# qc-tum/TNC

Hardware: NVIDIA H100
Metric: pairwise contractions/sec (effective ZGEMM TFLOP/s in zgemm_tflops) (higher is better)
Workload: dtype f64

## Files before the change

### tnc_b200/csrc/crt.cu

```cuda
#include "internal.h"
#include "sm90.h"
#include <cuda.h>
#include <algorithm>
#include <cmath>
#include <cstdio>
#include <cstdlib>

namespace tncb {

constexpr int CRT_MAX_MOD = 20;
static const int kModuli[CRT_MAX_MOD] = {256, 253, 251, 249, 247, 245, 241, 239, 233, 229,
                                         227, 223, 211, 199, 197, 193, 191, 181, 179, 173};
constexpr int CRT_BT = 128;
constexpr int CRT_BKB = WG_BKB;
#ifndef CRT_RING3_STAGES
#define CRT_RING3_STAGES 3
#endif
#ifndef CRT_RING3_BK
#define CRT_RING3_BK 128
#endif
#ifndef CRT_RING4_STAGES
#define CRT_RING4_STAGES 5
#endif
#ifndef CRT_RING4_BK
// ... 112 lines not shown
  unsigned long long mv[RES_ROWS_C * RES_K_C / 256];
#pragma unroll
  for (int it = 0; it < RES_ROWS_C * RES_K_C / 256; it++) {
    int r, k;
    crt_tile_coord(it * 256 + tid, lk, r, k);
    const long long orow = s_offr[r], ok = s_offk[k];
    mv[it] = 0ull;
    if (orow >= 0 && ok >= 0) {
      const double2 v = __ldg(src + orow + ok);
      mv[it] = max((unsigned long long)__double_as_longlong(fabs(v.x)), (unsigned long long)__double_as_longlong(fabs(v.y)));
    }
  }
  int cur_r = -1;
  unsigned long long cur_m = 0ull;
#pragma unroll
  for (int it = 0; it < RES_ROWS_C * RES_K_C / 256; it++) {
    int r, k;
    crt_tile_coord(it * 256 + tid, lk, r, k);
    unsigned long long m = mv[it];
    for (int d = 1; d < (1 << lk); d <<= 1) m = max(m, __shfl_xor_sync(0xffffffffu, m, d));
    if (r != cur_r) {
      if (cur_m && (tid & ((1 << lk) - 1)) == 0) atomicMax(&s_max[cur_r], cur_m);
      cur_r = r; cur_m = 0ull;
    }
    cur_m = max(cur_m, m);
  }
  if (cur_m && (tid & ((1 << lk) - 1)) == 0) atomicMax(&s_max[cur_r], cur_m);
  __syncthreads();
  if (tid < RES_ROWS_C && row0 + tid < rows && s_max[tid] != 0ull) atomicMax(rowmax + row0 + tid, s_max[tid]);
}

__device__ __forceinline__ int crt_fix_byte(int s, int m) {
  if (s > 127) s -= m;
  else if (s < -128) s += m;
  return s;
}
constexpr int RES_ROWS = RES_ROWS_C, RES_K = RES_K_C, RES_RS = RES_K + RES_K / 8 + 1;
template <int COMPS, bool KARA>
__global__ void __launch_bounds__(256, 3)
crt_residue_kernel(const double2* __restrict__ src, const long long* __restrict__ off_row, const long long* __restrict__ off_k,
                   long long rows, long long K, long long rowsP, long long Kp, const unsigned long long* __restrict__ rowmax, int bits, int lk,
                   const __grid_constant__ CrtTables T, int8_t* __restrict__ planes) {
  extern __shared__ __align__(16) unsigned char res_smem_raw[];
  double2* tile = reinterpret_cast<double2*>(res_smem_raw);
  __shared__ double s_scale[RES_ROWS];
  __shared__ long long s_offr[RES_ROWS], s_offk[RES_K];
  __shared__ double s_inv[CRT_MAX_MOD];
  __shared__ int s_mod[CRT_MAX_MOD];
  const long long row0 = (long long)blockIdx.x * RES_ROWS, k0 = (long long)blockIdx.y * RES_K;
  const int tid = threadIdx.x;
  const double two_a = scalbn(1.0, bits);
  if (tid >= 64 && tid < 64 + CRT_MAX_MOD) { s_inv[tid - 64] = T.inv_mod[tid - 64]; s_mod[tid - 64] = T.mod[tid - 64]; }
  if (tid < RES_ROWS) {
    const long long r = row0 + tid;
    const int e = r < rows ? crt_exp_from_bits(rowmax[r]) : 0;
    s_scale[tid] = (e == kExpNonFinite) ? 0.0 : scalbn(1.0, -e);
    s_offr[tid] = r < rows ? __ldg(off_row + r) : -1;
  } else if (tid >= 128) {
    const int k = tid - 128;
    s_offk[k] = k0 + k < K ? __ldg(off_k + k0 + k) : -1;
  }
  __syncthreads();
  double2 vv[RES_ROWS * RES_K / 256];
#pragma unroll
  for (int it = 0; it < RES_ROWS * RES_K / 256; it++) {
    int r, k;
    crt_tile_coord(it * 256 + tid, lk, r, k);
    const long long orow = s_offr[r], ok = s_offk[k];
    vv[it] = make_double2(0.0, 0.0);
    if (orow >= 0 && ok >= 0) vv[it] = __ldg(src + orow + ok);
  }
#pragma unroll
  for (int it = 0; it < RES_ROWS * RES_K / 256; it++) {
    int r, k;
    crt_tile_coord(it * 256 + tid, lk, r, k);
    const double sc = s_scale[r];
    double2 v = vv[it];
    v.x = trunc(v.x * sc * two_a);
    v.y = trunc(v.y * sc * two_a);
    if (sc == 0.0) { v.x = 0.0; v.y = 0.0; }
    tile[r * RES_RS + k + (k >> 3)] = v;
  }
  __syncthreads();
  const int r = tid >> 3;
  if (row0 + r >= rows) return;
  const double RMAGIC = 6755399441055744.0;
  const long long plane_stride = rowsP * Kp;
#pragma unroll 1
  for (int pass = 0; pass < 2; pass++) {
    const int g = (tid & 7) + 8 * pass;
    double xr[8], xi[8];
    int lr[8], li[8];
#pragma unroll
    for (int j = 0; j < 8; j++) {
      const double2 v = tile[r * RES_RS + g * 9 + j];
      xr[j] = v.x; xi[j] = v.y;
      lr[j] = (int)__double2ll_rn(v.x); li[j] = (int)__double2ll_rn(v.y);
    }
    int8_t* dst = planes + (row0 + r) * Kp + k0 + g * 8;
    const int nmod = T.nmod;
#pragma unroll 1
    for (int i = 0; i < nmod; i++) {
      const int m = s_mod[i];
      const double inv = s_inv[i];
      uint32_t wr[2] = {0, 0}, wi[2] = {0, 0}, ws[2] = {0, 0};
#pragma unroll
      for (int j = 0; j < 8; j++) {
        const int qr = __double2loint(fma(xr[j], inv, RMAGIC));
        const int qi = __double2loint(fma(xi[j], inv, RMAGIC));
        const int rr = lr[j] - qr * m, ri = li[j] - qi * m;
        constexpr uint32_t sel[4] = {0x3214u, 0x3240u, 0x3410u, 0x4210u};
        wr[j >> 2] = __byte_perm(wr[j >> 2], (uint32_t)rr, sel[j & 3]);
        wi[j >> 2] = __byte_perm(wi[j >> 2], (uint32_t)ri, sel[j & 3]);
        if (KARA) ws[j >> 2] = __byte_perm(ws[j >> 2], (uint32_t)crt_fix_byte(rr + ri, m), sel[j & 3]);
      }
      int8_t* d = dst + (long long)i * (KARA ? 3 : COMPS) * plane_stride;
      if (KARA) {
        *reinterpret_cast<uint2*>(d) = make_uint2(wr[0], wr[1]);
        *reinterpret_cast<uint2*>(d + plane_stride) = make_uint2(wi[0], wi[1]);
        *reinterpret_cast<uint2*>(d + 2 * plane_stride) = make_uint2(ws[0], ws[1]);
      } else if (COMPS == 2) {
        *reinterpret_cast<uint2*>(d) = make_uint2(wr[0], wr[1]);
        *reinterpret_cast<uint2*>(d + plane_stride) = make_uint2(wi[0], wi[1]);
      } else {
        *reinterpret_cast<uint2*>(d) = make_uint2(__vneg4(wi[0]), __vneg4(wi[1]));
        *reinterpret_cast<uint2*>(d + plane_stride) = make_uint2(wr[0], wr[1]);
        *reinterpret_cast<uint2*>(d + 2 * plane_stride) = make_uint2(wi[0], wi[1]);
      }
    }
  }
}

struct CrtGemmArgs {
  int8_t* R;
  int Np, Mp;
  int tiles_n, tiles_m, tile_m;
  int nmod, nkc, kb_per_chunk, num_kb;
  int total_items;
  int group;
  int negmod[CRT_MAX_MOD];
  int magic[CRT_MAX_MOD];
};

struct CrtItem { int mod_i, prod, kc, n0, m0; };
template <bool KARA>
__device__ __forceinline__ CrtItem crt_decode(const CrtGemmArgs& p, int item) {
  const int tiles = p.tiles_n * p.tiles_m;
  const int mk = item / tiles, t = item - mk * tiles;
  CrtItem it;
  const int mp = mk / p.nkc;
  it.kc = mk - mp * p.nkc;
  it.mod_i = KARA ? mp / 3 : mp; it.prod = KARA ? mp - it.mod_i * 3 : 0;
  const int per_band = p.group * p.tiles_m;
  const int band = t / per_band, first = band * p.group;
  const int gsize = min(p.group, p.tiles_n - first);
  const int r = t - band * per_band;
  it.n0 = (first + r % gsize) * CRT_BT;
  it.m0 = (r / gsize) * p.tile_m;
  return it;
}

template <bool KARA>
__global__ void __launch_bounds__(WG_THREADS, 1)
crt_gemm_kernel(const __grid_constant__ CUtensorMap mapB, const __grid_constant__ CUtensorMap mapA,
                const __grid_constant__ CrtGemmArgs p) {
  constexpr int STAGES = CrtRing<KARA>::STAGES, BK = CrtRing<KARA>::BK, SUB = CRT_BKB / BK;
  using Stage = typename CrtRing<KARA>::Stage;
  extern __shared__ __align__(1024) uint8_t crt_smem_raw[];
  uint8_t* smem = reinterpret_cast<uint8_t*>((reinterpret_cast<uintptr_t>(crt_smem_raw) + 1023) & ~(uintptr_t)1023);
  __shared__ uint64_t full_bar[STAGES], empty_bar[STAGES];
  const int wg = threadIdx.x >> 7, tid = threadIdx.x & 127;

  if (threadIdx.x == 0) {
    for (int s = 0; s < STAGES; s++) { wg_mbar_init(&full_bar[s], 1); wg_mbar_init(&empty_bar[s], 2); }
    asm volatile("fence.mbarrier_init.release.cluster;" ::: "memory");
  }
  __syncthreads();

  if (wg == 0) {
    wg_setmaxnreg_producer();
    if (tid != 0) return;
    int it = 0;
    for (int item = blockIdx.x; item < p.total_items; item += gridDim.x) {
      const CrtItem w = crt_decode<KARA>(p, item);
      const int kb0 = w.kc * p.kb_per_chunk, kb1 = min(p.num_kb, kb0 + p.kb_per_chunk);
      const int rowB = (KARA ? w.mod_i * 3 + w.prod : w.mod_i * 2) * p.Np + w.n0;
      const int rowA = (KARA ? w.mod_i * 3 + w.prod : w.mod_i * 3) * p.Mp + w.m0;
      for (int ks = kb0 * SUB; ks < kb1 * SUB; ks++, it++) {
        uint8_t* st = wg_produce_begin<STAGES, KARA, BK>(smem, full_bar, empty_bar, it);
        uint64_t* bar = &full_bar[it % STAGES];
        const int kx = ks * BK;
        uint8_t* a = st + Stage::A;
        wg_tma_2d(&mapB, bar, st, kx, rowB);
        if (KARA) {
          wg_tma_2d(&mapA, bar, a, kx, rowA);
          wg_tma_2d(&mapA, bar, a + Stage::TILE, kx, rowA + WG_ROWS);
        } else {
          wg_tma_2d(&mapB, bar, st + Stage::B1, kx, rowB + p.Np);
          wg_tma_2d(&mapA, bar, a, kx, rowA);
          wg_tma_2d(&mapA, bar, a + Stage::TILE, kx, rowA + p.Mp);
          wg_tma_2d(&mapA, bar, a + 2 * Stage::TILE, kx, rowA + 2 * p.Mp);
        }
      }
    }
  } else {
    wg_setmaxnreg_consumer();
    const int c = wg - 1, wq = tid >> 5, lane = tid & 31;
    const int q = lane & 3;
    const bool q0 = q & 1, q1 = q & 2;
    WgRing<STAGES, KARA, BK> ring{smem, full_bar, empty_bar};
    uint32_t acc[128];
#pragma unroll
    for (int i = 0; i < 128; i++) acc[i] = 0u;
    for (int item = blockIdx.x; item < p.total_items; item += gridDim.x) {
      const CrtItem w = crt_decode<KARA>(p, item);
      const int kb0 = w.kc * p.kb_per_chunk, kb1 = min(p.num_kb, kb0 + p.kb_per_chunk);
      bool first = true;
      for (int ks = kb0 * SUB; ks < kb1 * SUB; ks++) ring.mma_stage(acc, c, first, tid == 0);
      ring.drain(tid == 0);
      const int negm = p.negmod[w.mod_i], magic = p.magic[w.mod_i];
      int8_t* row_base[2];
#pragma unroll
      for (int h = 0; h < 2; h++) {
        const long long n = (long long)w.n0 + c * 64 + wq * 16 + (lane >> 2) + 8 * h;
        row_base[h] = KARA ? p.R + ((long long)((w.mod_i * p.nkc + w.kc) * 3 + w.prod) * p.Np + n) * p.Mp + w.m0
                           : p.R + ((long long)((w.mod_i * p.nkc + w.kc) * 2) * p.Np + n) * p.Mp + w.m0;
      }
#pragma unroll
      for (int i = 0; i < 4; i++) {
#pragma unroll
        for (int h = 0; h < 2; h++) {
          uint32_t x[4];
#pragma unroll
          for (int k = 0; k < 4; k++) {
            uint32_t u = 0;
#pragma unroll
            for (int jj = 0; jj < 2; jj++) {
#pragma unroll
              for (int e = 0; e < 2; e++) {
                const int a = (int)acc[4 * (8 * i + 2 * k + jj) + 2 * h + e];
                int t = __mulhi(a, magic) * negm + a;
                if (t > 127) t += negm;
                u |= (((uint32_t)t & 0xffu) ^ 0x80u) << (8 * (2 * jj + e));
              }
            }
            x[k] = u;
          }
          const uint32_t r0 = __shfl_xor_sync(0xffffffffu, q0 ? x[0] : x[1], 1);
          const uint32_t r1 = __shfl_xor_sync(0xffffffffu, q0 ? x[2] : x[3], 1);
          const uint32_t a0 = q0 ? r0 : x[0], a1 = q0 ? x[1] : r0;
          const uint32_t b0 = q0 ? r1 : x[2], b1 = q0 ? x[3] : r1;
          const uint32_t g0 = __shfl_xor_sync(0xffffffffu, q1 ? a0 : b0, 2);
          const uint32_t g1 = __shfl_xor_sync(0xffffffffu, q1 ? a1 : b1, 2);
          const uint32_t k0 = q1 ? b0 : a0, k1 = q1 ? b1 : a1;
          const uint32_t y0 = q1 ? g0 : k0, y1 = q1 ? g1 : k1, y2 = q1 ? k0 : g0, y3 = q1 ? k1 : g1;
          const uint4 v = make_uint4(__byte_perm(y0, y1, 0x5410), __byte_perm(y2, y3, 0x5410),
                                     __byte_perm(y0, y1, 0x7632), __byte_perm(y2, y3, 0x7632));
          const int cc = 4 * i + q;
          int8_t* dst = KARA ? row_base[h] + cc * 16
                             : row_base[h] + (i >= 2 ? (long long)p.Np * p.Mp : 0LL) + (cc & 7) * 16;
          *reinterpret_cast<uint4*>(dst) = v;
        }
      }
    }
  }
}

struct CrtReconArgs {
  const int8_t* R;
  double2* C;
  const unsigned long long* max_n;
  const unsigned long long* max_m;
  long long rows, cols, ldc;
  long long Np, Mp;
  int nkc;
};

template <bool ONE_CHUNK, bool KARA>
__global__ void __launch_bounds__(256, 4)
crt_reconstruct_kernel(const __grid_constant__ CrtReconArgs a, const __grid_constant__ CrtTables T) {
  const long long cols4 = a.Mp >> 2;
  const long long idx = (long long)blockIdx.x * blockDim.x + threadIdx.x;
  const long long n = idx / cols4, m4 = (idx - n * cols4) * 4;
  if (n >= a.rows || m4 >= a.cols) return;
  double s1r[4], s2r[4], s1i[4], s2i[4];
#pragma unroll
  for (int j = 0; j < 4; j++) { s1r[j] = s2r[j] = s1i[j] = s2i[j] = 0.0; }
  const long long plane = a.Np * a.Mp;
  const int8_t* base = a.R + n * a.Mp + m4;
  const double bias = 4503599627370496.0 + (KARA ? 256.0 : 128.0) * (double)a.nkc;
  const double bias_i = 4503599627370496.0 + (KARA ? 384.0 : 128.0) * (double)a.nkc;
#pragma unroll 8
  for (int i = 0; i < T.nmod; i++) {
    uint32_t ur[4], ui[4];
    if (KARA) {
#pragma unroll
      for (int j = 0; j < 4; j++) { ur[j] = 0; ui[j] = 0; }
      for (int c = 0; c < (ONE_CHUNK ? 1 : a.nkc); c++) {
        const int8_t* pk = base + (long long)((i * a.nkc + c) * 3) * plane;
        const uint32_t w1 = __ldg(reinterpret_cast<const uint32_t*>(pk));
        const uint32_t w2 = __ldg(reinterpret_cast<const uint32_t*>(pk + plane));
        const uint32_t w3 = __ldg(reinterpret_cast<const uint32_t*>(pk + 2 * plane));
#pragma unroll
        for (int j = 0; j < 4; j++) {
          const uint32_t k1 = __byte_perm(w1, 0, 0x4440 + j), k2 = __byte_perm(w2, 0, 0x4440 + j);
          ur[j] += 256u + k1 - k2;
          ui[j] += 512u + __byte_perm(w3, 0, 0x4440 + j) - k1 - k2;
        }
      }
    } else if (ONE_CHUNK) {
      const uint32_t wr = __ldg(reinterpret_cast<const uint32_t*>(base + (long long)(i * 2) * plane));
      const uint32_t wi = __ldg(reinterpret_cast<const uint32_t*>(base + (long long)(i * 2 + 1) * plane));
#pragma unroll
      for (int j = 0; j < 4; j++) { ur[j] = __byte_perm(wr, 0, 0x4440 + j); ui[j] = __byte_perm(wi, 0, 0x4440 + j); }
    } else {
#pragma unroll
      for (int j = 0; j < 4; j++) { ur[j] = 0; ui[j] = 0; }
      for (int c = 0; c < a.nkc; c++) {
        const int8_t* pr = base + (long long)((i * a.nkc + c) * 2) * plane;
        const uint32_t wr = __ldg(reinterpret_cast<const uint32_t*>(pr));
        const uint32_t wi = __ldg(reinterpret_cast<const uint32_t*>(pr + plane));
#pragma unroll
        for (int j = 0; j < 4; j++) { ur[j] += __byte_perm(wr, 0, 0x4440 + j); ui[j] += __byte_perm(wi, 0, 0x4440 + j); }
      }
    }
    const double r1 = T.rho1[i], r2 = T.rho2[i];
#pragma unroll
    for (int j = 0; j < 4; j++) {
      const double dr = __hiloint2double(0x43300000, (int)ur[j]) - bias;
      const double di = __hiloint2double(0x43300000, (int)ui[j]) - bias_i;
      s1r[j] = fma(dr, r1, s1r[j]); s2r[j] = fma(dr, r2, s2r[j]);
      s1i[j] = fma(di, r1, s1i[j]); s2i[j] = fma(di, r2, s2i[j]);
    }
  }
  const int en = crt_exp_from_bits(a.max_n[n]);
  double2* dst = a.C + n * a.ldc + m4;
  const double RMAGIC = 6755399441055744.0;
#pragma unroll
  for (int j = 0; j < 4; j++) {
    if (m4 + j >= a.cols) break;
    const int em = crt_exp_from_bits(a.max_m[m4 + j]);
    double2 out;
    if (en == kExpNonFinite || em == kExpNonFinite) {
      out = make_double2(__longlong_as_double(0x7ff8000000000000LL), __longlong_as_double(0x7ff8000000000000LL));
    } else {
      const double qr = ((s1r[j] + s2r[j]) + RMAGIC) - RMAGIC;
      const double qi = ((s1i[j] + s2i[j]) + RMAGIC) - RMAGIC;
      const double fr = (s1r[j] - qr) + s2r[j], fi = (s1i[j] - qi) + s2i[j];
      out = make_double2(scalbn(fr * T.p_scaled, en + em), scalbn(fi * T.p_scaled, en + em));
    }
    dst[j] = out;
  }
}

typedef CUresult (*EncodeTiledFn)(CUtensorMap*, CUtensorMapDataType, cuuint32_t, void*, const cuuint64_t*, const cuuint64_t*,
                                  const cuuint32_t*, const cuuint32_t*, CUtensorMapInterleave, CUtensorMapSwizzle,
                                  CUtensorMapL2promotion, CUtensorMapFloatOOBfill);
static EncodeTiledFn get_encode() {
  static EncodeTiledFn fn = nullptr;
  static bool tried = false;
  if (!tried) {
    tried = true;
    cudaDriverEntryPointQueryResult q;
    void* p = nullptr;
    if (cudaGetDriverEntryPoint("cuTensorMapEncodeTiled", &p, cudaEnableDefault, &q) == cudaSuccess) fn = (EncodeTiledFn)p;
  }
  return fn;
}
template <int BK>
int wg_make_map(CUtensorMap* m, void* ptr, uint64_t rows, uint64_t kbytes) {
  static_assert(BK == 128 || BK == 64, "SWIZZLE_128B or SWIZZLE_64B");
  EncodeTiledFn enc = get_encode();
  if (!enc) return fail(TNCB_ERR_CUDA, "cuTensorMapEncodeTiled is not available");
  cuuint64_t dims[2] = {kbytes, rows};
  cuuint64_t strides[1] = {kbytes};
  cuuint32_t box[2] = {(cuuint32_t)BK, (cuuint32_t)WG_ROWS};
  cuuint32_t estr[2] = {1, 1};
  CUresult r = enc(m, CU_TENSOR_MAP_DATA_TYPE_UINT8, 2, ptr, dims, strides, box, estr, CU_TENSOR_MAP_INTERLEAVE_NONE,
                   BK == 128 ? CU_TENSOR_MAP_SWIZZLE_128B : CU_TENSOR_MAP_SWIZZLE_64B, CU_TENSOR_MAP_L2_PROMOTION_L2_256B,
                   CU_TENSOR_MAP_FLOAT_OOB_FILL_NONE);
  if (r != CUDA_SUCCESS) return fail(TNCB_ERR_CUDA, "cuTensorMapEncodeTiled failed: " + std::to_string((int)r));
  return TNCB_OK;
}
template int wg_make_map<128>(CUtensorMap*, void*, uint64_t, uint64_t);
template int wg_make_map<64>(CUtensorMap*, void*, uint64_t, uint64_t);

static inline long long round_up_ll(long long x, long long a) { return (x + a - 1) / a * a; }


int launch_k1_crt(tncb_ctx* ctx, const PairPlan& P, const double2* A, const double2* B, double2* C,
                  const long long* offAm, const long long* offBn, const long long* offAk, const long long* offBk) {
  int nmod, bits_a, bits_b;
  const int want = ctx->crt_tol > 0.0 ? crt_bits_for_tolerance(P.K, ctx->crt_tol) : ctx->crt_bits;
  crt_choose(P.K, want, ctx->crt_nmod_force, &nmod, &bits_a, &bits_b);
  CrtTables T;
  crt_make_tables(nmod, bits_a, bits_b, T);
  cudaStream_t st = ctx->stream;
  const long long Kp = round_up_ll(P.K, CRT_BKB);
  const int num_kb = (int)(Kp / CRT_BKB);
  const int ctas_max = std::max(1, ctx->sm_count);
  const bool kara = ctx->crt_products == 3 || (ctx->crt_products == 0 && Kp >= ctx->crt_kara_min_k);
  const int TM = kara ? 2 * CRT_BT : CRT_BT;
  const int NPB = kara ? 3 : 2, NPR = kara ? 3 : 2;
  const long long tiles_total = round_up_ll(P.N, CRT_BT) / CRT_BT * (round_up_ll(P.M, TM) / TM);
  int nkc = (int)((Kp + CRT_KCHUNK_MAX - 1) / CRT_KCHUNK_MAX);
  {
    const long long items = tiles_total * nmod * (kara ? 3 : 1);
    const long long want = ctas_max;
    if (items * nkc < want) nkc = (int)std::min<long long>((want + items - 1) / items, std::max(1, num_kb / 8));
    nkc = std::max(1, std::min(nkc, 32));
  }
  int kb_per_chunk = (num_kb + nkc - 1) / nkc;
  nkc = (num_kb + kb_per_chunk - 1) / kb_per_chunk;
  if ((long long)kb_per_chunk * CRT_BKB > CRT_KCHUNK_MAX) return fail(TNCB_ERR_UNSUPPORTED, "K too long for the int8 engine");

  const size_t budget = ctx->crt_ws_bytes;
  long long pn = round_up_ll(P.N, CRT_BT), pm = round_up_ll(P.M, TM);
  auto ws_bytes = [&](long long n_, long long m_) {
    return (size_t)nmod * (size_t)Kp * (size_t)(NPB * n_ + 3 * m_) + (size_t)nmod * nkc * NPR * (size_t)n_ * (size_t)m_;
  };
  while (ws_bytes(pn, pm) > budget && (pm > TM || pn > CRT_BT)) {
    if (pm >= pn && pm > TM) pm = round_up_ll(pm / 2, TM);
    else if (pn > CRT_BT) pn = round_up_ll(pn / 2, CRT_BT);
    else pm = round_up_ll(pm / 2, TM);
  }
  const size_t bytesB = (size_t)nmod * NPB * pn * Kp, bytesA = (size_t)nmod * 3 * pm * Kp;
  const size_t bytesR = (size_t)nmod * nkc * NPR * pn * pm;
  const size_t bytesE = (size_t)(pn + pm) * sizeof(unsigned long long);
  void *pb = nullptr, *pa = nullptr, *pr = nullptr, *pe = nullptr;
  int rc;
  if ((rc = ctx->arena.alloc(bytesB, &pb))) return rc;
  if ((rc = ctx->arena.alloc(bytesA, &pa))) { ctx->arena.free(pb, bytesB); return rc; }
  if ((rc = ctx->arena.alloc(bytesR, &pr))) { ctx->arena.free(pb, bytesB); ctx->arena.free(pa, bytesA); return rc; }
  if ((rc = ctx->arena.alloc(bytesE, &pe))) { ctx->arena.free(pb, bytesB); ctx->arena.free(pa, bytesA); ctx->arena.free(pr, bytesR); return rc; }
  auto cleanup = [&]() { ctx->arena.free(pb, bytesB); ctx->arena.free(pa, bytesA); ctx->arena.free(pr, bytesR); ctx->arena.free(pe, bytesE); };
  unsigned long long* max_n = (unsigned long long*)pe;
  unsigned long long* max_m = max_n + pn;

  static bool attr_done_dev[64] = {false};
  bool& attr_done = attr_done_dev[ctx->device & 63];
  const int smem_gemm4 = CrtRing<false>::SMEM, smem_gemm3 = CrtRing<true>::SMEM;
  const int smem_res = RES_ROWS * RES_RS * (int)sizeof(double2);
  if (!attr_done) {
    cudaError_t e = cudaFuncSetAttribute(crt_gemm_kernel<false>, cudaFuncAttributeMaxDynamicSharedMemorySize, smem_gemm4);
    if (e == cudaSuccess) e = cudaFuncSetAttribute(crt_gemm_kernel<true>, cudaFuncAttributeMaxDynamicSharedMemorySize, smem_gemm3);
    if (e == cudaSuccess) e = cudaFuncSetAttribute(crt_residue_kernel<2, false>, cudaFuncAttributeMaxDynamicSharedMemorySize, smem_res);
    if (e == cudaSuccess) e = cudaFuncSetAttribute(crt_residue_kernel<3, false>, cudaFuncAttributeMaxDynamicSharedMemorySize, smem_res);
    if (e == cudaSuccess) e = cudaFuncSetAttribute(crt_residue_kernel<2, true>, cudaFuncAttributeMaxDynamicSharedMemorySize, smem_res);
    if (e == cudaSuccess) e = cudaFuncSetAttribute(crt_residue_kernel<3, true>, cudaFuncAttributeMaxDynamicSharedMemorySize, smem_res);
    if (e != cudaSuccess) { cleanup(); return fail(TNCB_ERR_CUDA, cudaGetErrorString(e)); }
    attr_done = true;
  }
  auto lane_split = [](const LegList& kl, bool k_is_b, const LegList& fl) {
    auto p2 = [](long long d) { int b = 0; while ((2LL << b) <= d && b < 5) b++; return b; };
    const long long ks = kl.n ? (k_is_b ? kl.sb[kl.n - 1] : kl.sa[kl.n - 1]) : (1LL << 62);
    const long long fs = fl.n ? fl.sa[fl.n - 1] : (1LL << 62);
    if (ks <= fs) return kl.n ? p2(kl.dim[kl.n - 1]) : 0;
    return 0;
  };
  const int lk_b = lane_split(P.k, true, P.n), lk_a = lane_split(P.k, false, P.m);
  ctx->last_int8_ops = 0.0; ctx->last_nmod = nmod; ctx->last_products = kara ? 3 : 4;
  bool timed = false;

  for (long long n0 = 0; n0 < P.N; n0 += pn) {
    const long long nrows = std::min(pn, P.N - n0);
    const long long Np = round_up_ll(nrows, CRT_BT);
    if (Np != nrows) cudaMemsetAsync(pb, 0, (size_t)nmod * NPB * Np * Kp, st);
    cudaMemsetAsync(max_n, 0, (size_t)nrows * sizeof(unsigned long long), st);
    {
      dim3 g((unsigned)((nrows + RES_ROWS - 1) / RES_ROWS), (unsigned)(Kp / RES_K));
      crt_rowmax_kernel<<<g, 256, 0, st>>>(B, offBn + n0, offBk, nrows, P.K, lk_b, max_n);
      if (kara) crt_residue_kernel<2, true><<<g, 256, smem_res, st>>>(B, offBn + n0, offBk, nrows, P.K, Np, Kp, max_n, bits_b, lk_b, T, (int8_t*)pb);
      else crt_residue_kernel<2, false><<<g, 256, smem_res, st>>>(B, offBn + n0, offBk, nrows, P.K, Np, Kp, max_n, bits_b, lk_b, T, (int8_t*)pb);
    }
    ctx->launches += 2;
    CUtensorMap mapB;
    if ((rc = kara ? wg_make_map<CrtRing<true>::BK>(&mapB, pb, (uint64_t)nmod * NPB * Np, (uint64_t)Kp)
                   : wg_make_map<CrtRing<false>::BK>(&mapB, pb, (uint64_t)nmod * NPB * Np, (uint64_t)Kp))) { cleanup(); return rc; }
    for (long long m0 = 0; m0 < P.M; m0 += pm) {
      const long long mcols = std::min(pm, P.M - m0);
      const long long Mp = round_up_ll(mcols, TM);
      if (Mp != mcols) cudaMemsetAsync(pa, 0, (size_t)nmod * 3 * Mp * Kp, st);
      cudaMemsetAsync(max_m, 0, (size_t)mcols * sizeof(unsigned long long), st);
      {
        dim3 g((unsigned)((mcols + RES_ROWS - 1) / RES_ROWS), (unsigned)(Kp / RES_K));
        crt_rowmax_kernel<<<g, 256, 0, st>>>(A, offAm + m0, offAk, mcols, P.K, lk_a, max_m);
        if (kara) crt_residue_kernel<3, true><<<g, 256, smem_res, st>>>(A, offAm + m0, offAk, mcols, P.K, Mp, Kp, max_m, bits_a, lk_a, T, (int8_t*)pa);
        else crt_residue_kernel<3, false><<<g, 256, smem_res, st>>>(A, offAm + m0, offAk, mcols, P.K, Mp, Kp, max_m, bits_a, lk_a, T, (int8_t*)pa);
      }
      ctx->launches += 2;
      CUtensorMap mapA;
      if ((rc = kara ? wg_make_map<CrtRing<true>::BK>(&mapA, pa, (uint64_t)nmod * 3 * Mp, (uint64_t)Kp)
                     : wg_make_map<CrtRing<false>::BK>(&mapA, pa, (uint64_t)nmod * 3 * Mp, (uint64_t)Kp))) { cleanup(); return rc; }
      CrtGemmArgs g;
      g.R = (int8_t*)pr; g.Np = (int)Np; g.Mp = (int)Mp;
      g.tiles_n = (int)(Np / CRT_BT); g.tiles_m = (int)(Mp / TM); g.tile_m = TM;
      g.nmod = nmod; g.nkc = nkc; g.kb_per_chunk = kb_per_chunk; g.num_kb = num_kb;
      const long long items = (long long)g.tiles_n * g.tiles_m * nmod * nkc * (kara ? 3 : 1);
      if (items > 0x7fffffffLL) { cleanup(); return fail(TNCB_ERR_UNSUPPORTED, "too many work items"); }
      g.total_items = (int)items;
      g.group = ctx->crt_group;
      for (int i = 0; i < CRT_MAX_MOD; i++) { g.negmod[i] = -T.mod[i]; g.magic[i] = T.magic[i]; }
      const unsigned grid = (unsigned)std::min<long long>(ctas_max, items);
      const double ops = 2.0 * (kara ? 3.0 : 4.0) * (double)nmod * (double)Np * (double)Mp * (double)Kp;
      const bool time_this = ctx->time_gemm == 2 || (ctx->time_gemm == 1 && !timed);
      if (time_this) gemm_timer_begin(ctx);
      if (kara) crt_gemm_kernel<true><<<grid, WG_THREADS, smem_gemm3, st>>>(mapB, mapA, g);
      else crt_gemm_kernel<false><<<grid, WG_THREADS, smem_gemm4, st>>>(mapB, mapA, g);
      cudaError_t e = cudaGetLastError();
      if (time_this) { gemm_timer_end(ctx, ops); timed = true; }
      if (e != cudaSuccess) { cleanup(); return fail(TNCB_ERR_CUDA, std::string("crt_gemm_kernel launch: ") + cudaGetErrorString(e)); }
      ctx->last_int8_ops += ops;
      CrtReconArgs r;
      r.R = (const int8_t*)pr; r.C = C + n0 * P.M + m0; r.max_n = max_n; r.max_m = max_m;
      r.rows = nrows; r.cols = mcols; r.ldc = P.M; r.Np = Np; r.Mp = Mp; r.nkc = nkc;
      const long long threads = nrows * (Mp / 4);
      const unsigned rg = (unsigned)((threads + 255) / 256);
      if (kara) {
        if (nkc == 1) crt_reconstruct_kernel<true, true><<<rg, 256, 0, st>>>(r, T);
        else crt_reconstruct_kernel<false, true><<<rg, 256, 0, st>>>(r, T);
      } else {
        if (nkc == 1) crt_reconstruct_kernel<true, false><<<rg, 256, 0, st>>>(r, T);
        else crt_reconstruct_kernel<false, false><<<rg, 256, 0, st>>>(r, T);
      }
      ctx->launches += 2;
    }
  }
  ctx->engine_count[4]++;
  cudaError_t e = cudaGetLastError();
  cleanup();
  if (e != cudaSuccess) return fail(TNCB_ERR_CUDA, std::string("K1' (CRT) launch: ") + cudaGetErrorString(e));
  return TNCB_OK;
}

}
```

### tnc_b200/csrc/internal.h

```cpp
#pragma once
#include <cstdint>
#include <cstddef>
#include <string>
#include <vector>
#include <map>
#include <cuda.h>
#include <cuda_runtime.h>
#include "../../include/tncb.h"

namespace tncb {

constexpr int kMaxLegs = 64;
constexpr int kMaxGroups = 40;

struct LegList {
  int n;
  int _pad;
  long long dim[kMaxGroups];
  long long sa[kMaxGroups];
  long long sb[kMaxGroups];
};

struct PairPlan {
  std::vector<uint64_t> out_legs, out_dims;
  long long M = 1, N = 1, K = 1;
  LegList m{}, n{}, k{};
  int kernel_class = 0;
  bool k2_big_is_a = true;
  bool a_kfast = false, b_kfast = true;
  double flops() const { return 8.0 * (double)M * (double)N * (double)K; }
  double bytes() const { return 16.0 * ((double)M * K + (double)K * N + (double)M * N); }
};

int plan_pair(int n_a, const uint64_t* a_legs, const uint64_t* a_dims,
              int n_b, const uint64_t* b_legs, const uint64_t* b_dims, PairPlan& plan);

void set_error(const std::string& msg);
int fail(int status, const std::string& msg);

struct Slab { char* base; size_t size; std::map<size_t, size_t> free_by_off; };

struct Arena {
  std::vector<Slab> slabs;
  size_t capacity_limit = 0;
  size_t reserved = 0, live = 0, peak = 0;
  size_t next_slab = (size_t)256 << 20;
  int alloc(size_t bytes, void** out);
  void free(void* p, size_t bytes);
  void release_all();
  size_t trim();
};

}

struct tncb_tensor {
  double2* ptr = nullptr;
  int rank = 0;
  uint64_t dims[tncb::kMaxLegs];
  uint64_t elems = 1;
  size_t bytes = 0;
  bool owned = true;
};

struct NcclApi;

struct tncb_ctx {
  int device = 0;
  cudaStream_t stream = nullptr;
  tncb::Arena arena;
  uint64_t launches = 0;
  int oz_slices = 8;
  int oz_engine = 0;
  long long oz_min_tiles = 96, oz_min_k = 1536;
  int crt_bits = 53; double crt_tol = 0.0; int crt_nmod_force = 0;
  long long crt_min_k = 256; double crt_min_mnk = 268435456.0;
  size_t crt_ws_bytes = (size_t)12 << 30; int crt_group = 8;
  double last_int8_ops = 0.0; int last_nmod = 0; int last_products = 0;
  int crt_products = 0;
  long long crt_kara_min_k = 2048;
  uint64_t engine_count[8] = {0, 0, 0, 0, 0, 0, 0, 0};
  int time_gemm = 0; cudaEvent_t gemm_ev0 = nullptr, gemm_ev1 = nullptr; bool gemm_ev_valid = false;
  std::vector<cudaEvent_t> gemm_pool; size_t gemm_used = 0; std::vector<double> gemm_ops;
  int sm_count = 132;
  void* stage_host = nullptr; size_t stage_bytes = 0;
  long long* tab = nullptr; size_t tab_elems = 0;
  bool tab_valid = false; tncb::LegList tab_m{}, tab_n{}, tab_k{};
  double2* partial = nullptr; size_t partial_elems = 0;
  double2* partial_override = nullptr; size_t partial_override_elems = 0;
  void* nccl_comm = nullptr; int world = 1, rank = 0;
  struct HostSlot { void* buf[3] = {nullptr, nullptr, nullptr}; size_t bytes[3] = {0, 0, 0};
                    cudaEvent_t in_done = nullptr, comp_done = nullptr, out_done = nullptr; bool busy = false; };
  HostSlot host_slot[3]; uint64_t host_jobs = 0;
  cudaStream_t h2d_stream = nullptr, d2h_stream = nullptr;
  std::vector<struct tncb_plan*> plans;
  struct CachedPlan { std::vector<uint64_t> key; struct tncb_plan* plan; };
  std::vector<CachedPlan> plan_cache;
  std::vector<struct tncb_angles*> angle_maps;
};

extern "C" void tncb_plan_release_device_state(struct tncb_plan* plan);
namespace tncb { void angles_release(struct tncb_angles* a, tncb_ctx* ctx); }

namespace tncb {
int launch_pair(tncb_ctx* ctx, const PairPlan& p, const double2* A, const double2* B, double2* C,
                int count = 1, long long stride = 0);
int launch_permute(tncb_ctx* ctx, const double2* in, double2* out, int rank,
                   const uint64_t* in_dims, const int* perm);
int launch_conj(tncb_ctx* ctx, double2* data, uint64_t elems);
int launch_add(tncb_ctx* ctx, double2* dst, const double2* src, uint64_t elems);
int ensure_tab(tncb_ctx* ctx, size_t elems);
int launch_k1_ozaki(tncb_ctx* ctx, const PairPlan& p, const double2* A, const double2* B, double2* C, int S,
                    const long long* offAm, const long long* offBn, const long long* offAk, const long long* offBk);

int launch_k1_crt(tncb_ctx* ctx, const PairPlan& p, const double2* A, const double2* B, double2* C,
                  const long long* offAm, const long long* offBn, const long long* offAk, const long long* offBk);
void crt_choose(long long K, int want_bits, int nmod_force, int* nmod, int* bits_a, int* bits_b);
int crt_bits_for_tolerance(long long K, double tol);
int crt_export_tables(int nmod, int* moduli, double* rho1, double* rho2, double* log2_product);

void gemm_timer_begin(tncb_ctx* ctx);
void gemm_timer_end(tncb_ctx* ctx, double ops);

int ensure_partial(tncb_ctx* ctx, size_t elems);
size_t k0_partial_elems(int sm_count, const PairPlan& p);

constexpr int kBatchGroups = 8;
struct CompactLegs { int n; int _pad; long long dim[kBatchGroups]; long long sa[kBatchGroups]; long long sb[kBatchGroups]; };
struct K0BatchItem {
  long long offA, offB, offC;
  long long M, N, K;
  int G, _pad;
  CompactLegs m, n, k;
};
bool k0_batch_eligible(int sm_count, const PairPlan& p);
int k0_batch_fill(int sm_count, const PairPlan& p, K0BatchItem* item);
int launch_k0_batch(tncb_ctx* ctx, const K0BatchItem* d_items, const int* d_block_start, int n_items, int total_blocks, char* ws,
                    int count = 1, long long stride = 0);

constexpr int kGradGroups = 8;
struct GradItem {
  long long src;
  long long dst;
  long long elems;
  int n, _pad;
  long long dim[kGradGroups];
  long long st[kGradGroups];
};
constexpr int kGradThreads = 256;
int launch_grad_gather(tncb_ctx* ctx, const GradItem* d_items, const long long* d_block_start, int n_items,
                       long long total_blocks, const char* ws, double2* out);
int launch_grad_gather_batch(tncb_ctx* ctx, const GradItem* d_items, const long long* d_block_start, int n_items,
                             long long total_blocks, const char* ws, long long stride, int n, double2* rows,
                             long long row_elems, double2* sum);

constexpr int kSliceGroups = 8, kSliceLegs = 8;
struct SliceItem {
  long long slot;
  long long full;
  long long elems;
  int n, ns;
  int from_scratch, _pad;
  long long dim[kSliceGroups];
  long long st[kSliceGroups];
  long long fst[kSliceGroups];
  unsigned long long sdiv[kSliceLegs], sdim[kSliceLegs];
  long long sst[kSliceLegs];
// ... 43 lines not shown
```

### tnc_b200/csrc/runtime.cu

```cuda
#include "internal.h"
#include <algorithm>
#include <cstdio>
#include <cstdlib>
#include <cstring>
#include <cmath>

namespace tncb {

static inline size_t round_up(size_t x, size_t a) { return (x + a - 1) / a * a; }

int Arena::alloc(size_t bytes, void** out) {
  bytes = round_up(std::max<size_t>(bytes, 256), 256);
  for (Slab& s : slabs) {
    for (auto it = s.free_by_off.begin(); it != s.free_by_off.end(); ++it) {
      if (it->second >= bytes) {
        size_t off = it->first, sz = it->second;
        s.free_by_off.erase(it);
        if (sz > bytes) s.free_by_off[off + bytes] = sz - bytes;
        *out = s.base + off;
        live += bytes; peak = std::max(peak, live);
        return TNCB_OK;
      }
    }
  }
// ... 38 lines not shown
      live -= bytes;
      return;
    }
  }
}

void Arena::release_all() {
  for (Slab& s : slabs) cudaFree(s.base);
  slabs.clear(); reserved = live = 0;
}

size_t Arena::trim() {
  size_t freed = 0;
  for (size_t i = 0; i < slabs.size();) {
    Slab& s = slabs[i];
    if (s.free_by_off.size() == 1 && s.free_by_off.begin()->first == 0 && s.free_by_off.begin()->second == s.size) {
      cudaFree(s.base);
      freed += s.size; reserved -= s.size;
      slabs.erase(slabs.begin() + i);
    } else i++;
  }
  if (slabs.empty()) next_slab = (size_t)256 << 20;
  return freed;
}

void gemm_timer_begin(tncb_ctx* ctx) {
  if (ctx->time_gemm == 1) cudaEventRecord(ctx->gemm_ev0, ctx->stream);
  else if (ctx->time_gemm == 2) {
    if (ctx->gemm_used + 2 > ctx->gemm_pool.size()) {
      cudaEvent_t a, b; cudaEventCreate(&a); cudaEventCreate(&b);
      ctx->gemm_pool.push_back(a); ctx->gemm_pool.push_back(b);
    }
    cudaEventRecord(ctx->gemm_pool[ctx->gemm_used], ctx->stream);
  }
}

void gemm_timer_end(tncb_ctx* ctx, double ops) {
  if (ctx->time_gemm == 1) { cudaEventRecord(ctx->gemm_ev1, ctx->stream); ctx->gemm_ev_valid = true; }
  else if (ctx->time_gemm == 2) {
    cudaEventRecord(ctx->gemm_pool[ctx->gemm_used + 1], ctx->stream);
    ctx->gemm_used += 2; ctx->gemm_ops.push_back(ops);
  }
}

int tensor_new(tncb_ctx* ctx, int rank, const uint64_t* dims, tncb_tensor** out) {
  if (rank < 0 || rank > kMaxLegs) return fail(TNCB_ERR_INVALID, "tensor rank out of range");
  tncb_tensor* t = new tncb_tensor();
  t->rank = rank; t->elems = 1;
  for (int i = 0; i < rank; i++) { t->dims[i] = dims[i]; t->elems *= dims[i]; }
  t->bytes = std::max<size_t>(t->elems * sizeof(double2), 16);
  void* p = nullptr;
  int rc = ctx->arena.alloc(t->bytes, &p);
  if (rc) { delete t; return rc; }
  t->ptr = (double2*)p;
  *out = t;
  return TNCB_OK;
}

}

using namespace tncb;

extern "C" {

int tncb_ctx_create(int device, size_t arena_bytes, tncb_ctx** out) {
  if (!out) return fail(TNCB_ERR_INVALID, "out is null");
  int count = 0;
  cudaError_t e = cudaGetDeviceCount(&count);
  if (e != cudaSuccess || count == 0) {
    cudaGetLastError();
    return fail(TNCB_ERR_CUDA, std::string("no CUDA device available (") + cudaGetErrorString(e) +
                                   "); libtncb200 has no CPU fallback");
  }
  if (device < 0 || device >= count) return fail(TNCB_ERR_INVALID, "device index out of range");
  TNCB_CUDA(cudaSetDevice(device));
  cudaDeviceProp prop;
  TNCB_CUDA(cudaGetDeviceProperties(&prop, device));
  if (prop.major != 9 || prop.minor != 0)
    return fail(TNCB_ERR_CUDA, std::string("device is sm_") + std::to_string(prop.major * 10 + prop.minor) +
                                   ", libtncb200 is built for sm_90a only");
  tncb_ctx* ctx = new tncb_ctx();
  ctx->device = device;
  ctx->sm_count = prop.multiProcessorCount;
  ctx->arena.capacity_limit = arena_bytes;
  if (const char* e = std::getenv("TNCB_OZAKI_SLICES")) ctx->oz_slices = std::max(0, std::min(8, atoi(e)));
  if (const char* e = std::getenv("TNCB_TCGEN05_ENGINE")) ctx->oz_engine = atoi(e) == 1 ? 1 : 0;
  if (const char* e = std::getenv("TNCB_CRT_MODULI")) ctx->crt_nmod_force = std::max(0, std::min(20, atoi(e)));
  if (const char* e = std::getenv("TNCB_CRT_PRODUCTS")) { const int v = atoi(e); ctx->crt_products = (v == 3 || v == 4) ? v : 0; }
  if (const char* e = std::getenv("TNCB_CRT_MIN_K3")) ctx->crt_kara_min_k = std::max(1, atoi(e));
  if (const char* e = std::getenv("TNCB_CRT_GROUP")) ctx->crt_group = std::max(1, atoi(e));
  if (const char* e = std::getenv("TNCB_CRT_WS_GB")) ctx->crt_ws_bytes = (size_t)std::max(1, atoi(e)) << 30;
  cudaError_t se = cudaStreamCreateWithFlags(&ctx->stream, cudaStreamNonBlocking);
  if (se != cudaSuccess) { delete ctx; return fail(TNCB_ERR_CUDA, cudaGetErrorString(se)); }
  cudaMemPool_t pool;
  if (cudaDeviceGetDefaultMemPool(&pool, device) == cudaSuccess) {
    uint64_t thr = UINT64_MAX;
    cudaMemPoolSetAttribute(pool, cudaMemPoolAttrReleaseThreshold, &thr);
  }
  *out = ctx;
  return TNCB_OK;
}

void tncb_ctx_destroy(tncb_ctx* ctx) {
  if (!ctx) return;
  cudaSetDevice(ctx->device);
  cudaStreamSynchronize(ctx->stream);
  for (auto& c : ctx->plan_cache) tncb_plan_destroy(c.plan);
  ctx->plan_cache.clear();
  while (!ctx->plans.empty()) tncb_plan_release_device_state(ctx->plans.back());
  while (!ctx->angle_maps.empty()) tncb::angles_release(ctx->angle_maps.back(), ctx);
  tncb_comm_destroy(ctx);
  if (ctx->tab) cudaFree(ctx->tab);
  if (ctx->partial) cudaFree(ctx->partial);
  if (ctx->stage_host) cudaFreeHost(ctx->stage_host);
  if (ctx->gemm_ev0) { cudaEventDestroy(ctx->gemm_ev0); cudaEventDestroy(ctx->gemm_ev1); }
  for (cudaEvent_t e : ctx->gemm_pool) cudaEventDestroy(e);
  if (ctx->h2d_stream) {
    cudaStreamSynchronize(ctx->h2d_stream); cudaStreamSynchronize(ctx->d2h_stream);
    for (auto& sl : ctx->host_slot) {
      for (int i = 0; i < 3; i++) if (sl.buf[i]) cudaFree(sl.buf[i]);
      cudaEventDestroy(sl.in_done); cudaEventDestroy(sl.comp_done); cudaEventDestroy(sl.out_done);
    }
    cudaStreamDestroy(ctx->h2d_stream); cudaStreamDestroy(ctx->d2h_stream);
  }
  ctx->arena.release_all();
  cudaStreamDestroy(ctx->stream);
  delete ctx;
}

int tncb_ctx_synchronize(tncb_ctx* ctx) {
  if (!ctx) return fail(TNCB_ERR_INVALID, "ctx is null");
  TNCB_CUDA(cudaSetDevice(ctx->device));
  TNCB_CUDA(cudaStreamSynchronize(ctx->stream));
  if (ctx->d2h_stream) {
    TNCB_CUDA(cudaStreamSynchronize(ctx->h2d_stream));
    TNCB_CUDA(cudaStreamSynchronize(ctx->d2h_stream));
    for (auto& sl : ctx->host_slot) sl.busy = false;
  }
  return TNCB_OK;
}

int tncb_contract_pair_host(tncb_ctx* ctx, int n_a, const uint64_t* a_legs, const uint64_t* a_dims, const double* host_a,
                            int n_b, const uint64_t* b_legs, const uint64_t* b_dims, const double* host_b, double* host_c) {
  if (!ctx || !host_a || !host_b || !host_c) return fail(TNCB_ERR_INVALID, "null argument");
  TNCB_CUDA(cudaSetDevice(ctx->device));
  PairPlan P;
  int rc = plan_pair(n_a, a_legs, a_dims, n_b, b_legs, b_dims, P);
  if (rc) return rc;
  size_t ea = 1, eb = 1;
  for (int i = 0; i < n_a; i++) ea *= a_dims[i];
  for (int i = 0; i < n_b; i++) eb *= b_dims[i];
  const size_t need[3] = {std::max<size_t>(ea * 16, 16), std::max<size_t>(eb * 16, 16), std::max<size_t>((size_t)(P.M * P.N) * 16, 16)};
  if (!ctx->h2d_stream) {
    TNCB_CUDA(cudaStreamCreateWithFlags(&ctx->h2d_stream, cudaStreamNonBlocking));
    TNCB_CUDA(cudaStreamCreateWithFlags(&ctx->d2h_stream, cudaStreamNonBlocking));
    for (auto& sl : ctx->host_slot) {
      TNCB_CUDA(cudaEventCreateWithFlags(&sl.in_done, cudaEventDisableTiming));
      TNCB_CUDA(cudaEventCreateWithFlags(&sl.comp_done, cudaEventDisableTiming));
      TNCB_CUDA(cudaEventCreateWithFlags(&sl.out_done, cudaEventDisableTiming));
    }
  }
  tncb_ctx::HostSlot& sl = ctx->host_slot[ctx->host_jobs % 3];
  if (sl.busy) TNCB_CUDA(cudaEventSynchronize(sl.out_done));
  for (int i = 0; i < 3; i++)
    if (sl.bytes[i] < need[i]) {
      if (sl.buf[i]) TNCB_CUDA(cudaFree(sl.buf[i]));
      sl.buf[i] = nullptr; sl.bytes[i] = 0;
      cudaError_t e = cudaMalloc(&sl.buf[i], need[i]);
      if (e != cudaSuccess) { cudaGetLastError(); return fail(TNCB_ERR_OOM, std::string("cudaMalloc (host pipeline): ") + cudaGetErrorString(e)); }
      sl.bytes[i] = need[i];
    }
  TNCB_CUDA(cudaMemcpyAsync(sl.buf[0], host_a, ea * 16, cudaMemcpyHostToDevice, ctx->h2d_stream));
  TNCB_CUDA(cudaMemcpyAsync(sl.buf[1], host_b, eb * 16, cudaMemcpyHostToDevice, ctx->h2d_stream));
// ... 298 lines not shown
```

Before: 5855.

## Retune CRT residue stores, batch reconstruct loads, size GEMM group from L2

The residue-plane writer now has 32 lanes cover a row with 4-byte stores, so a warp writes contiguous rows instead of scattered 8-byte chunks. The reconstruct kernel now issues the loads for up to eight moduli at once in the single-chunk case, lowers the minimum blocks per SM for the Karatsuba variant, and writes output with streaming stores. The GEMM tile-group size is now derived from the device L2 size instead of a fixed value, and the environment override for it is removed. The changes aim to improve coalescing, memory-level parallelism and L2 reuse, at the cost of more registers and losing the manual group tuning.

```diff
diff --git a/tnc_b200/csrc/crt.cu b/tnc_b200/csrc/crt.cu
--- a/tnc_b200/csrc/crt.cu
+++ b/tnc_b200/csrc/crt.cu
@@ -218,50 +218,46 @@
     tile[r * RES_RS + k + (k >> 3)] = v;
   }
   __syncthreads();
-  const int r = tid >> 3;
-  if (row0 + r >= rows) return;
   const double RMAGIC = 6755399441055744.0;
   const long long plane_stride = rowsP * Kp;
+  const int g = tid & 31;
+  const int nmod = T.nmod;
 #pragma unroll 1
-  for (int pass = 0; pass < 2; pass++) {
-    const int g = (tid & 7) + 8 * pass;
-    double xr[8], xi[8];
-    int lr[8], li[8];
-#pragma unroll
-    for (int j = 0; j < 8; j++) {
-      const double2 v = tile[r * RES_RS + g * 9 + j];
+  for (int pass = 0; pass < RES_ROWS / 8; pass++) {
+    const int r = (tid >> 5) + 8 * pass;
+    if (row0 + r >= rows) return;
+    double xr[4], xi[4];
+    int lr[4], li[4];
+#pragma unroll
+    for (int j = 0; j < 4; j++) {
+      const double2 v = tile[r * RES_RS + g * 4 + j + (g >> 1)];
       xr[j] = v.x; xi[j] = v.y;
       lr[j] = (int)__double2ll_rn(v.x); li[j] = (int)__double2ll_rn(v.y);
     }
-    int8_t* dst = planes + (row0 + r) * Kp + k0 + g * 8;
-    const int nmod = T.nmod;
+    int8_t* dst = planes + (row0 + r) * Kp + k0 + g * 4;
 #pragma unroll 1
     for (int i = 0; i < nmod; i++) {
       const int m = s_mod[i];
       const double inv = s_inv[i];
-      uint32_t wr[2] = {0, 0}, wi[2] = {0, 0}, ws[2] = {0, 0};
-#pragma unroll
-      for (int j = 0; j < 8; j++) {
+      uint32_t wr = 0, wi = 0, ws = 0;
+#pragma unroll
+      for (int j = 0; j < 4; j++) {
         const int qr = __double2loint(fma(xr[j], inv, RMAGIC));
         const int qi = __double2loint(fma(xi[j], inv, RMAGIC));
         const int rr = lr[j] - qr * m, ri = li[j] - qi * m;
         constexpr uint32_t sel[4] = {0x3214u, 0x3240u, 0x3410u, 0x4210u};
-        wr[j >> 2] = __byte_perm(wr[j >> 2], (uint32_t)rr, sel[j & 3]);
-        wi[j >> 2] = __byte_perm(wi[j >> 2], (uint32_t)ri, sel[j & 3]);
-        if (KARA) ws[j >> 2] = __byte_perm(ws[j >> 2], (uint32_t)crt_fix_byte(rr + ri, m), sel[j & 3]);
-      }
-      int8_t* d = dst + (long long)i * (KARA ? 3 : COMPS) * plane_stride;
+        wr = __byte_perm(wr, (uint32_t)rr, sel[j]);
+        wi = __byte_perm(wi, (uint32_t)ri, sel[j]);
+        if (KARA) ws = __byte_perm(ws, (uint32_t)crt_fix_byte(rr + ri, m), sel[j]);
+      }
+      uint32_t* d = reinterpret_cast<uint32_t*>(dst + (long long)i * (KARA ? 3 : COMPS) * plane_stride);
+      const long long ps = plane_stride / 4;
       if (KARA) {
-        *reinterpret_cast<uint2*>(d) = make_uint2(wr[0], wr[1]);
-        *reinterpret_cast<uint2*>(d + plane_stride) = make_uint2(wi[0], wi[1]);
-        *reinterpret_cast<uint2*>(d + 2 * plane_stride) = make_uint2(ws[0], ws[1]);
+        d[0] = wr; d[ps] = wi; d[2 * ps] = ws;
       } else if (COMPS == 2) {
-        *reinterpret_cast<uint2*>(d) = make_uint2(wr[0], wr[1]);
-        *reinterpret_cast<uint2*>(d + plane_stride) = make_uint2(wi[0], wi[1]);
+        d[0] = wr; d[ps] = wi;
       } else {
-        *reinterpret_cast<uint2*>(d) = make_uint2(__vneg4(wi[0]), __vneg4(wi[1]));
-        *reinterpret_cast<uint2*>(d + plane_stride) = make_uint2(wr[0], wr[1]);
-        *reinterpret_cast<uint2*>(d + 2 * plane_stride) = make_uint2(wi[0], wi[1]);
+        d[0] = __vneg4(wi); d[ps] = wr; d[2 * ps] = wi;
       }
     }
   }
@@ -413,8 +409,9 @@
 };
 
 template <bool ONE_CHUNK, bool KARA>
-__global__ void __launch_bounds__(256, 4)
+__global__ void __launch_bounds__(256, KARA ? 3 : 4)
 crt_reconstruct_kernel(const __grid_constant__ CrtReconArgs a, const __grid_constant__ CrtTables T) {
+  constexpr int NPR = KARA ? 3 : 2, RB = 8;
   const long long cols4 = a.Mp >> 2;
   const long long idx = (long long)blockIdx.x * blockDim.x + threadIdx.x;
   const long long n = idx / cols4, m4 = (idx - n * cols4) * 4;
@@ -426,47 +423,55 @@
   const int8_t* base = a.R + n * a.Mp + m4;
   const double bias = 4503599627370496.0 + (KARA ? 256.0 : 128.0) * (double)a.nkc;
   const double bias_i = 4503599627370496.0 + (KARA ? 384.0 : 128.0) * (double)a.nkc;
-#pragma unroll 8
-  for (int i = 0; i < T.nmod; i++) {
-    uint32_t ur[4], ui[4];
-    if (KARA) {
+  const int nmod = T.nmod;
+#pragma unroll 1
+  for (int i0 = 0; i0 < nmod; i0 += RB) {
+    uint32_t w[RB][NPR];
+    if (ONE_CHUNK) {
+#pragma unroll
+      for (int u = 0; u < RB; u++) {
+        if (i0 + u < nmod) {
+#pragma unroll
+          for (int p = 0; p < NPR; p++) w[u][p] = __ldg(reinterpret_cast<const uint32_t*>(base + (long long)((i0 + u) * NPR + p) * plane));
+        }
+      }
+    }
+#pragma unroll
+    for (int u = 0; u < RB; u++) {
+      const int i = i0 + u;
+      if (i >= nmod) break;
+      uint32_t ur[4], ui[4];
 #pragma unroll
       for (int j = 0; j < 4; j++) { ur[j] = 0; ui[j] = 0; }
       for (int c = 0; c < (ONE_CHUNK ? 1 : a.nkc); c++) {
-        const int8_t* pk = base + (long long)((i * a.nkc + c) * 3) * plane;
-        const uint32_t w1 = __ldg(reinterpret_cast<const uint32_t*>(pk));
-        const uint32_t w2 = __ldg(reinterpret_cast<const uint32_t*>(pk + plane));
-        const uint32_t w3 = __ldg(reinterpret_cast<const uint32_t*>(pk + 2 * plane));
+        uint32_t x[NPR];
+        if (ONE_CHUNK) {
+#pragma unroll
+          for (int p = 0; p < NPR; p++) x[p] = w[u][p];
+        } else {
+          const int8_t* pk = base + (long long)((i * a.nkc + c) * NPR) * plane;
+#pragma unroll
+          for (int p = 0; p < NPR; p++) x[p] = __ldg(reinterpret_cast<const uint32_t*>(pk + p * plane));
+        }
 #pragma unroll
         for (int j = 0; j < 4; j++) {
-          const uint32_t k1 = __byte_perm(w1, 0, 0x4440 + j), k2 = __byte_perm(w2, 0, 0x4440 + j);
-          ur[j] += 256u + k1 - k2;
-          ui[j] += 512u + __byte_perm(w3, 0, 0x4440 + j) - k1 - k2;
+          const uint32_t k1 = __byte_perm(x[0], 0, 0x4440 + j), k2 = __byte_perm(x[1], 0, 0x4440 + j);
+          if (KARA) {
+            ur[j] += 256u + k1 - k2;
+            ui[j] += 512u + __byte_perm(x[NPR - 1], 0, 0x4440 + j) - k1 - k2;
+          } else {
+            ur[j] += k1; ui[j] += k2;
+          }
         }
       }
-    } else if (ONE_CHUNK) {
-      const uint32_t wr = __ldg(reinterpret_cast<const uint32_t*>(base + (long long)(i * 2) * plane));
-      const uint32_t wi = __ldg(reinterpret_cast<const uint32_t*>(base + (long long)(i * 2 + 1) * plane));
-#pragma unroll
-      for (int j = 0; j < 4; j++) { ur[j] = __byte_perm(wr, 0, 0x4440 + j); ui[j] = __byte_perm(wi, 0, 0x4440 + j); }
-    } else {
-#pragma unroll
-      for (int j = 0; j < 4; j++) { ur[j] = 0; ui[j] = 0; }
-      for (int c = 0; c < a.nkc; c++) {
-        const int8_t* pr = base + (long long)((i * a.nkc + c) * 2) * plane;
-        const uint32_t wr = __ldg(reinterpret_cast<const uint32_t*>(pr));
-        const uint32_t wi = __ldg(reinterpret_cast<const uint32_t*>(pr + plane));
-#pragma unroll
-        for (int j = 0; j < 4; j++) { ur[j] += __byte_perm(wr, 0, 0x4440 + j); ui[j] += __byte_perm(wi, 0, 0x4440 + j); }
-      }
-    }
-    const double r1 = T.rho1[i], r2 = T.rho2[i];
-#pragma unroll
-    for (int j = 0; j < 4; j++) {
-      const double dr = __hiloint2double(0x43300000, (int)ur[j]) - bias;
-      const double di = __hiloint2double(0x43300000, (int)ui[j]) - bias_i;
-      s1r[j] = fma(dr, r1, s1r[j]); s2r[j] = fma(dr, r2, s2r[j]);
-      s1i[j] = fma(di, r1, s1i[j]); s2i[j] = fma(di, r2, s2i[j]);
+      const double r1 = T.rho1[i], r2 = T.rho2[i];
+#pragma unroll
+      for (int j = 0; j < 4; j++) {
+        const double dr = __hiloint2double(0x43300000, (int)ur[j]) - bias;
+        const double di = __hiloint2double(0x43300000, (int)ui[j]) - bias_i;
+        s1r[j] = fma(dr, r1, s1r[j]); s2r[j] = fma(dr, r2, s2r[j]);
+        s1i[j] = fma(di, r1, s1i[j]); s2i[j] = fma(di, r2, s2i[j]);
+      }
     }
   }
   const int en = crt_exp_from_bits(a.max_n[n]);
@@ -485,7 +490,7 @@
       const double fr = (s1r[j] - qr) + s2r[j], fi = (s1i[j] - qi) + s2i[j];
       out = make_double2(scalbn(fr * T.p_scaled, en + em), scalbn(fi * T.p_scaled, en + em));
     }
-    dst[j] = out;
+    __stcs(dst + j, out);
   }
 }
 
@@ -635,7 +640,8 @@
       const long long items = (long long)g.tiles_n * g.tiles_m * nmod * nkc * (kara ? 3 : 1);
       if (items > 0x7fffffffLL) { cleanup(); return fail(TNCB_ERR_UNSUPPORTED, "too many work items"); }
       g.total_items = (int)items;
-      g.group = ctx->crt_group;
+      const long long bt_tile_bytes = (long long)CRT_BT * Kp * (kara ? 1 : 2);
+      g.group = (int)std::max<long long>(1, std::min<long long>(g.tiles_n, ctx->l2_bytes / 2 / bt_tile_bytes));
       for (int i = 0; i < CRT_MAX_MOD; i++) { g.negmod[i] = -T.mod[i]; g.magic[i] = T.magic[i]; }
       const unsigned grid = (unsigned)std::min<long long>(ctas_max, items);
       const double ops = 2.0 * (kara ? 3.0 : 4.0) * (double)nmod * (double)Np * (double)Mp * (double)Kp;
diff --git a/tnc_b200/csrc/internal.h b/tnc_b200/csrc/internal.h
--- a/tnc_b200/csrc/internal.h
+++ b/tnc_b200/csrc/internal.h
@@ -74,7 +74,7 @@
   long long oz_min_tiles = 96, oz_min_k = 1536;
   int crt_bits = 53; double crt_tol = 0.0; int crt_nmod_force = 0;
   long long crt_min_k = 256; double crt_min_mnk = 268435456.0;
-  size_t crt_ws_bytes = (size_t)12 << 30; int crt_group = 8;
+  size_t crt_ws_bytes = (size_t)12 << 30;
   double last_int8_ops = 0.0; int last_nmod = 0; int last_products = 0;
   int crt_products = 0;
   long long crt_kara_min_k = 2048;
@@ -82,6 +82,7 @@
   int time_gemm = 0; cudaEvent_t gemm_ev0 = nullptr, gemm_ev1 = nullptr; bool gemm_ev_valid = false;
   std::vector<cudaEvent_t> gemm_pool; size_t gemm_used = 0; std::vector<double> gemm_ops;
   int sm_count = 132;
+  long long l2_bytes = 50LL << 20;
   void* stage_host = nullptr; size_t stage_bytes = 0;
   long long* tab = nullptr; size_t tab_elems = 0;
   bool tab_valid = false; tncb::LegList tab_m{}, tab_n{}, tab_k{};
diff --git a/tnc_b200/csrc/runtime.cu b/tnc_b200/csrc/runtime.cu
--- a/tnc_b200/csrc/runtime.cu
+++ b/tnc_b200/csrc/runtime.cu
@@ -144,13 +144,13 @@
   tncb_ctx* ctx = new tncb_ctx();
   ctx->device = device;
   ctx->sm_count = prop.multiProcessorCount;
+  ctx->l2_bytes = prop.l2CacheSize;
   ctx->arena.capacity_limit = arena_bytes;
   if (const char* e = std::getenv("TNCB_OZAKI_SLICES")) ctx->oz_slices = std::max(0, std::min(8, atoi(e)));
   if (const char* e = std::getenv("TNCB_TCGEN05_ENGINE")) ctx->oz_engine = atoi(e) == 1 ? 1 : 0;
   if (const char* e = std::getenv("TNCB_CRT_MODULI")) ctx->crt_nmod_force = std::max(0, std::min(20, atoi(e)));
   if (const char* e = std::getenv("TNCB_CRT_PRODUCTS")) { const int v = atoi(e); ctx->crt_products = (v == 3 || v == 4) ? v : 0; }
   if (const char* e = std::getenv("TNCB_CRT_MIN_K3")) ctx->crt_kara_min_k = std::max(1, atoi(e));
-  if (const char* e = std::getenv("TNCB_CRT_GROUP")) ctx->crt_group = std::max(1, atoi(e));
   if (const char* e = std::getenv("TNCB_CRT_WS_GB")) ctx->crt_ws_bytes = (size_t)std::max(1, atoi(e)) << 30;
   cudaError_t se = cudaStreamCreateWithFlags(&ctx->stream, cudaStreamNonBlocking);
   if (se != cudaSuccess) { delete ctx; return fail(TNCB_ERR_CUDA, cudaGetErrorString(se)); }
```

New measurement: 6164 (median of 6 runs). 1.05x the previous value.
